# deezer/musicFPaugment

Measured on AMD Instinct MI355X. Metric: 8s/8kHz clips/sec (STFT+UNet+peak-pick), higher is better.
Workload: dtype bf16x3 (fp32 operands split into bf16 hi+lo, fp32 accumulate); 1 GPU; STFT(512/256,f64) -> UNet(1,1) eval forward (bf16x3 MFMA, formula weights) -> Audfprint peak-pick; 8 s / 8 kHz clips, 257x251 spectrograms; parallelism=clip-sharded x1, no data-path collective

## Files before the change

### musicfpaugment_amd/csrc/unet_wd16.hip

```cpp
#include "mfpa_common.h"
#include "mfpa_conv_tile.h"
#include "mfpa_unet_args.h"

namespace {

using namespace mfpa_tile;
using mfpa_unet::ConvArgs;

constexpr int wd16_bn(int wmw) { return 32 * (8 / wmw); }
constexpr bool wd16_persist(bool rows, int wmw, bool side, bool plain) { return wmw == 4 || (!rows && !side) || plain; }
template <int PH, int PW, bool IN16>
struct Wd16Lds {
  static constexpr int THREADS = 512;
  static constexpr int SPP = IN16 ? KC / 8 : KC / 4;
  static constexpr int HPW = PW + 2, HPH = PH + 2, HP = HPW * HPH;
  static constexpr int A_F4 = (HP * SPP + THREADS - 1) / THREADS;
  static constexpr int HPS = A_F4 * (THREADS / SPP);
  static constexpr int PLANE = ((HPS * 16 + 255) / 256) * 256;
  static constexpr int HLS = 4 * PLANE + 256;
  static constexpr int STAGE = 2 * HLS;
  static constexpr int TBL = 2 * A_F4 * THREADS;
  static constexpr int TBL_BYTES = 2 * ((HP * (KC / 4) + THREADS - 1) / THREADS) * THREADS * (int)sizeof(unsigned);
  static constexpr int RED = 2 * 256;
  static constexpr int epi_floats(int wmw) { return 2 * wd16_bn(wmw) + 64; }
  static constexpr int fixed_bytes(int wmw) { return 2 * STAGE + TBL_BYTES + epi_floats(wmw) * (int)sizeof(float); }
  __host__ __device__ static constexpr int plane_off(int hl, int kg) { return hl * HLS + kg * PLANE + (kg >> 1) * 128; }
  static_assert(TBL * (int)sizeof(unsigned) <= TBL_BYTES, "the kernel's table fits the launcher's");
};
static_assert(Wd16Lds<8, 32, false>::fixed_bytes(2) == 125184 && Wd16Lds<16, 16, false>::fixed_bytes(2) == 125184 &&
              Wd16Lds<8, 32, true>::fixed_bytes(2) == 125184 && Wd16Lds<16, 16, true>::fixed_bytes(2) == 125184, "LDS of the 128-channel tiles");
static_assert(Wd16Lds<8, 32, false>::fixed_bytes(4) == 124672 && Wd16Lds<8, 32, true>::fixed_bytes(4) == 124672, "LDS of the 64-channel tiles");


template <int PH, int PW, bool ROWS, int WMW = 2, bool SIDE = false, bool PLAIN = false, bool IN16 = false, bool AFF16 = false>
__global__ __launch_bounds__(512, 1) void conv_wd16_kernel(ConvArgs a) {
  static_assert(!IN16 || PLAIN, "a bf16 source feeds the plain-bf16 products");
  using G = Wd16Lds<PH, PW, IN16>;
  constexpr int SPP = G::SPP, HPW = G::HPW, HP = G::HP, A_F4 = G::A_F4, HLS = G::HLS, STAGE = G::STAGE, TBL = G::TBL;
  constexpr int ESZ = IN16 ? 2 : 4;
  constexpr int THREADS = G::THREADS, BN = wd16_bn(WMW), WPXW = 256 / WMW, TAPS = 9;
  static_assert((WMW == 2 || WMW == 4) && (!ROWS || WMW == 2), "wave grid");
  constexpr int BM = PH * PW;
  static_assert(BM == 256 && (PW == 32 || PW == 16), "two waves of 128 pixels: eight 16-pixel tiles each");
  constexpr int PT = WPXW / 16;
  static_assert(A_F4 <= TAPS - 3, "one halo staging slot per tap, taps 2 .. 7");

  extern __shared__ __attribute__((aligned(16))) char smem[];
  const int tid = threadIdx.x, lane = tid & 63, wave = tid >> 6;
  const int wm = wave % WMW, wn = __builtin_amdgcn_readfirstlane(wave / WMW);
  const int p = lane & 15, g = lane >> 4;

  constexpr bool PERSIST = wd16_persist(ROWS, WMW, SIDE, PLAIN);
  const int n0 = blockIdx.y * BN;
  const int Cin = a.C0 + a.C1;
  const int nchunks = Cin / KC;
  const int ntiles = a.tiles_x * a.tiles_y * a.B;

  const int aq = tid % SPP;
  unsigned* const aoffs0 = reinterpret_cast<unsigned*>(smem + 2 * STAGE);
#pragma unroll
  for (int it = 0; it < A_F4; ++it) {
    const int pix = tid / SPP + it * (THREADS / SPP);
    const int py = pix / HPW - 1, px = pix % HPW - 1;
    aoffs0[it * THREADS + tid] = (unsigned)((py * a.W + px) * a.C0 + (KC / SPP) * aq) * (unsigned)ESZ;
    aoffs0[(A_F4 + it) * THREADS + tid] = (unsigned)(((py - a.oy1) * a.W1 + (px - a.ox1)) * a.C1 + (KC / SPP) * aq) * (unsigned)ESZ;
  }
  const unsigned clip0 = (unsigned)a.H * (unsigned)a.W * (unsigned)a.C0 * (unsigned)ESZ, clip1 = (unsigned)a.H1 * (unsigned)a.W1 * (unsigned)a.C1 * (unsigned)ESZ;
  struct Tile { int b, y0, x0p; unsigned ain; unsigned t0, t1; };
  auto make_tile = [&](int t) __attribute__((always_inline)) {
    Tile T;
    int bx = __builtin_amdgcn_readfirstlane(t);
    const int tx = bx % a.tiles_x; bx /= a.tiles_x;
    const int ty = bx % a.tiles_y; bx /= a.tiles_y;
    T.b = bx; T.y0 = ty * PH; T.x0p = tx * PW; T.ain = 0;
    T.t0 = (unsigned)((T.y0 * a.W + T.x0p) * a.C0) * (unsigned)ESZ;
    T.t1 = (unsigned)((T.y0 * a.W1 + T.x0p) * a.C1) * (unsigned)ESZ;
#pragma unroll
    for (int it = 0; it < A_F4; ++it) {
      const int pix = tid / SPP + it * (THREADS / SPP);
      const int gy = T.y0 + pix / HPW - 1, gx = T.x0p + pix % HPW - 1;
      const bool in = pix < HP && gy >= 0 && gy < a.H && gx >= 0 && gx < a.W;
      const int y1 = gy - a.oy1, x1 = gx - a.ox1;
      const bool in1 = in && y1 >= 0 && y1 < a.H1 && x1 >= 0 && x1 < a.W1;
      T.ain |= (in ? 1u : 0u) << it | (in1 ? 1u : 0u) << (8 + it);
    }
    return T;
  };
  auto clip_rsrc = [&](const float* base, int b, unsigned clip_bytes) __attribute__((always_inline)) {
    const char* pb = reinterpret_cast<const char*>(base) + (size_t)b * clip_bytes;
    return __builtin_amdgcn_make_buffer_rsrc(const_cast<char*>(pb), 0, base != nullptr ? (int)clip_bytes : 0, 0x00020000);
  };
  int tile = blockIdx.x;
  Tile S = make_tile(tile);
  int eb = S.b, ey0 = S.y0, ex0p = S.x0p;
  float* aff = reinterpret_cast<float*>(smem + 2 * STAGE + TBL * sizeof(unsigned));
  if (a.in_scale0 != nullptr) {
    for (int i = tid; i < a.C0; i += THREADS) {
      aff[i] = a.in_scale0[i];
      aff[a.C0 + i] = a.in_shift0[i];
    }
    __syncthreads();
  }
  float* const epi = aff + (a.in_scale0 ? 2 * a.C0 : 0) + (a.w1x1 ? G::RED : 0);
  for (int i = tid; i < BN; i += THREADS) {
    epi[i] = a.scale ? a.scale[n0 + i] : 1.f;
    epi[BN + i] = a.shift ? a.shift[n0 + i] : 0.f;
  }
  if (a.w1x1 != nullptr && tid < 64) epi[2 * BN + tid] = a.w1x1[tid];
  constexpr int AHALF = (A_F4 + 1) / 2, AREGS = ROWS ? AHALF : A_F4;
  f32x4 areg[AREGS];
  auto load_a_range = [&](int chunk, auto FIRST, auto COUNT) __attribute__((always_inline)) {
    constexpr int first = decltype(FIRST)::value, count = decltype(COUNT)::value;
    const int c0 = chunk * KC;
    const bool from0 = c0 < a.C0;
    const auto rs = clip_rsrc(from0 ? a.x0 : a.x1, S.b, from0 ? clip0 : clip1);
    const unsigned toff = from0 ? S.t0 + (unsigned)c0 * (unsigned)ESZ : S.t1 + (unsigned)(c0 - a.C0) * (unsigned)ESZ;
    const unsigned* ao = aoffs0 + (from0 ? 0 : A_F4 * THREADS) + tid;
#pragma unroll
    for (int it = first; it < first + count && it < A_F4; ++it)
      areg[it % AREGS] = __builtin_bit_cast(f32x4, __builtin_amdgcn_raw_buffer_load_b128(rs, (int)(ao[it * THREADS] + toff), 0, 0));
  };
  auto load_a = [&](int chunk) __attribute__((always_inline)) {
    load_a_range(chunk, std::integral_constant<int, 0>{}, std::integral_constant<int, AREGS>{});
  };
  auto preload_offsets = [&](int chunk) __attribute__((always_inline)) {
    const unsigned* ao = aoffs0 + (chunk * KC < a.C0 ? 0 : A_F4 * THREADS) + tid;
#pragma unroll
    for (int it = 0; it < A_F4; ++it) areg[it % AREGS][0] = __uint_as_float(ao[it * THREADS]);
  };
  auto load_a_pre = [&](int chunk) __attribute__((always_inline)) {
    const int c0 = chunk * KC;
    const bool from0 = c0 < a.C0;
    const auto rs = clip_rsrc(from0 ? a.x0 : a.x1, S.b, from0 ? clip0 : clip1);
    const unsigned toff = from0 ? S.t0 + (unsigned)c0 * (unsigned)ESZ : S.t1 + (unsigned)(c0 - a.C0) * (unsigned)ESZ;
#pragma unroll
    for (int it = 0; it < A_F4; ++it)
      areg[it % AREGS] = __builtin_bit_cast(f32x4, __builtin_amdgcn_raw_buffer_load_b128(rs, (int)(__float_as_uint(areg[it % AREGS][0]) + toff), 0, 0));
  };
  auto split_slot = [&](auto IT, int chunk, char* stage) __attribute__((always_inline)) {
    constexpr int it = decltype(IT)::value;
    const int pix = tid / SPP + it * (THREADS / SPP);
    const int c0 = chunk * KC;
    const bool inside = (S.ain >> ((c0 < a.C0 ? 0 : 8) + it)) & 1u;
    f32x4 v = areg[it % AREGS];
    if (!inside) v = f32x4{0.f, 0.f, 0.f, 0.f};
    if constexpr (IN16) {
      if (AFF16 && a.in_scale0 != nullptr && c0 < a.C0 && inside) {
        float f[8];
#pragma unroll
        for (int k = 0; k < 4; ++k) {
          const unsigned u = __float_as_uint(v[k]);
          f[2 * k] = __uint_as_float(u << 16);
          f[2 * k + 1] = __uint_as_float(u & 0xffff0000u);
        }
        const float* scp = aff + c0 + 8 * aq;
        const float* shp = aff + a.C0 + c0 + 8 * aq;
        const f32x4 sc0 = *reinterpret_cast<const f32x4*>(scp), sc1 = *reinterpret_cast<const f32x4*>(scp + 4);
        const f32x4 sh0 = *reinterpret_cast<const f32x4*>(shp), sh1 = *reinterpret_cast<const f32x4*>(shp + 4);
#pragma unroll
        for (int k = 0; k < 8; ++k) {
          const float y = f[k] * (k < 4 ? sc0[k & 3] : sc1[k & 3]) + (k < 4 ? sh0[k & 3] : sh1[k & 3]);
          f[k] = y > 0.f ? y : 0.f;
        }
        if (a.drop_thresh) {
          const int gy = S.y0 + pix / HPW - 1, gx = S.x0p + pix % HPW - 1;
          const unsigned long long e0 = (((unsigned long long)S.b * a.H + gy) * a.W + gx) * a.C0 + c0 + 8 * aq;
#pragma unroll
          for (int k = 0; k < 8; ++k) f[k] = mfpa_keep(a.drop_seed, a.drop_thresh, e0 + k) ? f[k] * a.drop_scale : 0.f;
        }
#pragma unroll
        for (int k = 0; k < 4; ++k) {
          bf16x2 h2;
          h2[0] = (__bf16)f[2 * k];
          h2[1] = (__bf16)f[2 * k + 1];
          v[k] = __builtin_bit_cast(float, h2);
        }
      }
      *reinterpret_cast<f32x4*>(stage + G::plane_off(0, aq) + pix * 16) = v;
      if constexpr (SIDE && AFF16) {
        const int py = pix / HPW, px = pix % HPW;
        if (a.x0_bf16 != nullptr && c0 < a.C0 && inside && py >= 1 && py <= PH && px >= 1 && px <= PW && blockIdx.y == 0) {
          const size_t e = (size_t)S.b * a.H * a.W * a.C0 + ((aoffs0[it * THREADS + tid] + S.t0) >> 1) + c0;
          *reinterpret_cast<f32x4*>(a.x0_bf16 + e) = v;
        }
      }
      return;
    }
    if (a.in_scale0 != nullptr && c0 < a.C0 && inside) {
      const f32x4 sc = *reinterpret_cast<const f32x4*>(aff + c0 + 4 * aq);
      const f32x4 sh = *reinterpret_cast<const f32x4*>(aff + a.C0 + c0 + 4 * aq);
      v = v * sc + sh;
#pragma unroll
      for (int k = 0; k < 4; ++k) v[k] = v[k] > 0.f ? v[k] : 0.f;
      if (a.drop_thresh) {
        const int gy = S.y0 + pix / HPW - 1, gx = S.x0p + pix % HPW - 1;
        const unsigned long long e0 = (((unsigned long long)S.b * a.H + gy) * a.W + gx) * a.C0 + c0 + 4 * aq;
#pragma unroll
        for (int k = 0; k < 4; ++k) v[k] = mfpa_keep(a.drop_seed, a.drop_thresh, e0 + k) ? v[k] * a.drop_scale : 0.f;
      }
    }
    bf16x4 hi, lo;
#pragma unroll
    for (int k = 0; k < 4; ++k) {
      hi[k] = (__bf16)v[k];
      lo[k] = (__bf16)(v[k] - (float)hi[k]);
    }
    char* at = stage + G::plane_off(0, aq >> 1) + pix * 16 + 8 * (aq & 1);
    *reinterpret_cast<bf16x4*>(at) = hi;
    if constexpr (!PLAIN) *reinterpret_cast<bf16x4*>(at + HLS) = lo;
    if constexpr (SIDE) {
      const int py = pix / HPW, px = pix % HPW;
      const bool interior = inside && py >= 1 && py <= PH && px >= 1 && px <= PW && blockIdx.y == 0;
      if (a.x0_bf16 != nullptr && c0 < a.C0 && interior) {
        const size_t e = (size_t)S.b * a.H * a.W * a.C0 + ((aoffs0[it * THREADS + tid] + S.t0) >> 2) + c0;
        *reinterpret_cast<bf16x4*>(a.x0_bf16 + e) = hi;
      }
      if (a.x1_bf16 != nullptr && c0 >= a.C0 && interior) {
        const size_t e = (size_t)S.b * a.H1 * a.W1 * a.C1 + ((aoffs0[(A_F4 + it) * THREADS + tid] + S.t1) >> 2) + (c0 - a.C0);
        *reinterpret_cast<bf16x4*>(a.x1_bf16 + e) = hi;
      }
    }
  };

  bf16x8 wq[3][2][2];
  auto w_frag = [&](int tap, int chunk) __attribute__((always_inline)) {
    return reinterpret_cast<const char*>(a.w) +
           ((((size_t)tap * nchunks + chunk) * (size_t)(a.Cout / 16) + (size_t)(n0 / 16 + 2 * wn)) << 11) + lane * 16;
  };
  auto load_w = [&](int chunk, int tap, auto SLOT) __attribute__((always_inline)) {
    constexpr int slot = decltype(SLOT)::value;
    const char* wb = w_frag(tap, chunk);
    wq[slot][0][0] = *reinterpret_cast<const bf16x8*>(wb);
    if constexpr (!PLAIN) wq[slot][0][1] = *reinterpret_cast<const bf16x8*>(wb + 1024);
    wq[slot][1][0] = *reinterpret_cast<const bf16x8*>(wb + 2048);
    if constexpr (!PLAIN) wq[slot][1][1] = *reinterpret_cast<const bf16x8*>(wb + 3072);
  };

  struct XFrags { bf16x8 h[4], l[4]; };
  XFrags fx0, fx1;
  const int xbase = (((wm * WPXW + p) / PW) * HPW + ((wm * WPXW + p) % PW)) * 16 + G::plane_off(0, g);
  auto tile_disp = [](int pt) { return (PW == 32) ? ((pt >> 1) * HPW + (pt & 1) * 16) * 16 : pt * HPW * 16; };
  auto read_x = [&](XFrags& f, const char* stage, int tap_off, int half) __attribute__((always_inline)) {
#pragma unroll
    for (int i = 0; i < 4; ++i) {
      const char* r = stage + xbase + tile_disp(4 * half + i) + tap_off;
      if constexpr (!PLAIN) f.l[i] = *reinterpret_cast<const bf16x8*>(r + HLS);
      f.h[i] = *reinterpret_cast<const bf16x8*>(r);
    }
  };
  floatx4 acc[2][PT];
#pragma unroll
  for (int ct = 0; ct < 2; ++ct)
#pragma unroll
    for (int pt = 0; pt < PT; ++pt) acc[ct][pt] = floatx4{0.f, 0.f, 0.f, 0.f};
  auto mfma_half = [&](const XFrags& f, const bf16x8 (&w)[2][2], int half) __attribute__((always_inline)) {
    if constexpr (!PLAIN) {
#pragma unroll
    for (int ct = 0; ct < 2; ++ct)
#pragma unroll
      for (int i = 0; i < 4; ++i) acc[ct][4 * half + i] = __builtin_amdgcn_mfma_f32_16x16x32_bf16(w[ct][1], f.h[i], acc[ct][4 * half + i], 0, 0, 0);
#pragma unroll
    for (int ct = 0; ct < 2; ++ct)
#pragma unroll
      for (int i = 0; i < 4; ++i) acc[ct][4 * half + i] = __builtin_amdgcn_mfma_f32_16x16x32_bf16(w[ct][0], f.l[i], acc[ct][4 * half + i], 0, 0, 0);
    }
#pragma unroll
    for (int ct = 0; ct < 2; ++ct)
#pragma unroll
      for (int i = 0; i < 4; ++i) acc[ct][4 * half + i] = __builtin_amdgcn_mfma_f32_16x16x32_bf16(w[ct][0], f.h[i], acc[ct][4 * half + i], 0, 0, 0);
  };
  using S0 = std::integral_constant<int, 0>;
  using S1 = std::integral_constant<int, 1>;
  constexpr int N_R = PLAIN ? 4 : 8, N_M = PLAIN ? 8 : 24;
  constexpr int N_W = PLAIN ? 2 : 4;
  auto tap_body = [&](auto TAP, int chunk) __attribute__((always_inline)) {
    constexpr int tap = decltype(TAP)::value;
    constexpr int ntap = (tap + 1) % TAPS;
    constexpr int tap_off = ((tap / 3) * HPW + (tap % 3)) * 16, ntap_off = ((ntap / 3) * HPW + (ntap % 3)) * 16;
    const int chunk_n = chunk + 1 < nchunks ? chunk + 1 : (PERSIST ? 0 : chunk);
    const char* cur = smem + (chunk & 1) * STAGE;
    const char* nxt = (tap == TAPS - 1) ? smem + ((chunk + 1) & 1) * STAGE : cur;
    read_x(fx1, cur, tap_off, 1);
    mfma_half(fx0, wq[tap % 3], 0);
    load_w((tap + 2 >= TAPS) ? chunk_n : chunk, (tap + 2) % TAPS, std::integral_constant<int, (tap + 2) % 3>{});
    pin_reads<N_M - 1, N_R>();
    constexpr int used_a = pin_read_slots(N_M - 1, N_R);
    __builtin_amdgcn_sched_group_barrier(0x008, 1, 0);
    __builtin_amdgcn_sched_group_barrier(0x020, N_W, 0);
    if constexpr (N_M - used_a - 1 > 0) __builtin_amdgcn_sched_group_barrier(0x008, N_M - used_a - 1, 0);
    __builtin_amdgcn_sched_barrier(0);
    if (tap == TAPS - 1) {
      __syncthreads();
      __builtin_amdgcn_sched_barrier(0);
    }
    if (tap == 0) load_a_pre(chunk_n);
    if (tap == TAPS - 1) preload_offsets(PERSIST ? (chunk + 2 < nchunks ? chunk + 2 : chunk + 1 < nchunks ? 0 : 1 < nchunks ? 1 : 0)
                                                 : (chunk + 2 < nchunks ? chunk + 2 : chunk + 1 < nchunks ? chunk + 1 : chunk));
    read_x(fx0, nxt, ntap_off, 0);
    mfma_half(fx1, wq[tap % 3], 1);
    if constexpr (tap >= 2 && tap - 2 < A_F4) {
      split_slot(std::integral_constant<int, tap - 2>{}, chunk_n, smem + ((chunk + 1) & 1) * STAGE);
#pragma unroll
      for (int i = 0; i < N_R; ++i) {
        __builtin_amdgcn_sched_group_barrier(0x008, 1, 0);
        __builtin_amdgcn_sched_group_barrier(0x100, 1, 0);
        __builtin_amdgcn_sched_group_barrier(0x002, 2, 0);
      }
#pragma unroll
      for (int i = 0; i < 2; ++i) {
        __builtin_amdgcn_sched_group_barrier(0x008, 2, 0);
        __builtin_amdgcn_sched_group_barrier(0x002, 4, 0);
        __builtin_amdgcn_sched_group_barrier(0x200, 1, 0);
      }
      if constexpr (N_M - N_R - 4 > 0) __builtin_amdgcn_sched_group_barrier(0x008, N_M - N_R - 4, 0);
    } else {
      pin_reads<N_M, N_R>();
      if constexpr (N_M - pin_read_slots(N_M, N_R) > 0) __builtin_amdgcn_sched_group_barrier(0x008, N_M - pin_read_slots(N_M, N_R), 0);
    }
    __builtin_amdgcn_sched_barrier(0);
  };

  auto tap_body4 = [&](auto TAP, auto PAR, int chunk) __attribute__((always_inline)) {
    constexpr int tap = decltype(TAP)::value, par = (decltype(PAR)::value + tap) & 1;
    constexpr int ntap = (tap + 1) % TAPS;
    constexpr int ntap_off = ((ntap / 3) * HPW + (ntap % 3)) * 16;
    const int chunk_n = chunk + 1 < nchunks ? chunk + 1 : 0;
    const char* cur = smem + (chunk & 1) * STAGE;
    const char* nxt = (tap == TAPS - 1) ? smem + ((chunk + 1) & 1) * STAGE : cur;
    if (tap == TAPS - 1) {
      __syncthreads();
      __builtin_amdgcn_sched_barrier(0);
    }
    if (tap == 0) load_a_pre(chunk_n);
    if (tap == TAPS - 1) preload_offsets(chunk + 2 < nchunks ? chunk + 2 : chunk + 1 < nchunks ? 0 : 1 < nchunks ? 1 : 0);
    read_x(par ? fx0 : fx1, nxt, ntap_off, 0);
    mfma_half(par ? fx1 : fx0, wq[tap % 3], 0);
    load_w((tap + 2 >= TAPS) ? chunk_n : chunk, (tap + 2) % TAPS, std::integral_constant<int, (tap + 2) % 3>{});
    if constexpr (tap >= 2 && tap - 2 < A_F4) {
      split_slot(std::integral_constant<int, tap - 2>{}, chunk_n, smem + ((chunk + 1) & 1) * STAGE);
#pragma unroll
      for (int i = 0; i < N_R; ++i) {
        __builtin_amdgcn_sched_group_barrier(0x008, 1, 0);
        __builtin_amdgcn_sched_group_barrier(0x100, 1, 0);
        __builtin_amdgcn_sched_group_barrier(0x002, 2, 0);
      }
#pragma unroll
      for (int i = 0; i < N_W; ++i) {
        if constexpr (!PLAIN) __builtin_amdgcn_sched_group_barrier(0x008, 1, 0);
        __builtin_amdgcn_sched_group_barrier(0x020, 1, 0);
        __builtin_amdgcn_sched_group_barrier(0x002, 2, 0);
      }
#pragma unroll
      for (int i = 0; i < 2; ++i) {
        __builtin_amdgcn_sched_group_barrier(0x008, 2, 0);
        __builtin_amdgcn_sched_group_barrier(0x002, 4, 0);
        __builtin_amdgcn_sched_group_barrier(0x200, 1, 0);
      }
      if constexpr (N_M - N_R - 8 > 0) __builtin_amdgcn_sched_group_barrier(0x008, N_M - N_R - 8, 0);
    } else {
#pragma unroll
      for (int i = 0; i < N_R; ++i) {
        __builtin_amdgcn_sched_group_barrier(0x008, 1, 0);
        __builtin_amdgcn_sched_group_barrier(0x100, 1, 0);
      }
#pragma unroll
      for (int i = 0; i < N_W; ++i) {
        __builtin_amdgcn_sched_group_barrier(0x008, 1, 0);
        __builtin_amdgcn_sched_group_barrier(0x020, 1, 0);
      }
      if constexpr (N_M - N_R - N_W > 0) __builtin_amdgcn_sched_group_barrier(0x008, N_M - N_R - N_W, 0);
    }
    __builtin_amdgcn_sched_barrier(0);
  };

  constexpr int R = BM / 2 / PW, HV = PW / 16;
  bf16x8 wr[2][3][2][2];
  constexpr int NU = (R + 2) * HV, NB = (PW == 32) ? 4 : 5;
  static_assert(NU % NB == 0, "static ring indices");
  auto load_wr1 = [&](int chunk, auto DX, auto PAR, auto DY) __attribute__((always_inline)) {
    constexpr int dx = decltype(DX)::value, par = decltype(PAR)::value, dy = decltype(DY)::value;
    const char* wb = w_frag(dy * 3 + dx, chunk);
    wr[par][dy][0][0] = *reinterpret_cast<const bf16x8*>(wb);
    if constexpr (!PLAIN) wr[par][dy][0][1] = *reinterpret_cast<const bf16x8*>(wb + 1024);
    wr[par][dy][1][0] = *reinterpret_cast<const bf16x8*>(wb + 2048);
    if constexpr (!PLAIN) wr[par][dy][1][1] = *reinterpret_cast<const bf16x8*>(wb + 3072);
  };
  struct XUnit { bf16x8 h, l; };
  XUnit xu[NB];
  auto read_unit = [&](XUnit& f, const char* stage, int u, int dx) __attribute__((always_inline)) {
    const char* r = stage + xbase + ((u / HV) * HPW + (u % HV) * 16 + dx) * 16;
    if constexpr (!PLAIN) f.l = *reinterpret_cast<const bf16x8*>(r + HLS);
    f.h = *reinterpret_cast<const bf16x8*>(r);
  };
  auto mfma_unit = [&](auto U, const XUnit& f, auto PAR) __attribute__((always_inline)) {
    constexpr int h = decltype(U)::value / HV, hv = decltype(U)::value % HV, par = decltype(PAR)::value;
#pragma unroll
    for (int term = PLAIN ? 2 : 0; term < 3; ++term)
#pragma unroll
      for (int dy = 0; dy < 3; ++dy) {
        if (h - dy < 0 || h - dy >= R) continue;
#pragma unroll
        for (int ct = 0; ct < 2; ++ct) {
          floatx4& c = acc[ct][(h - dy) * HV + hv];
          c = __builtin_amdgcn_mfma_f32_16x16x32_bf16(wr[par][dy][ct][term == 0 ? 1 : 0], term == 1 ? f.l : f.h, c, 0, 0, 0);
        }
      }
  };
  auto unit_mfmas = [](int u) { const int h = u / HV; int n = 0; for (int dy = 0; dy < 3; ++dy) n += (h - dy >= 0 && h - dy < R) ? 1 : 0; return n * (PLAIN ? 2 : 6); };
  constexpr int BARU = NU - NB + 1;
  constexpr int SA = NU / 2, SB = BARU - AHALF;
  static_assert(SA + AHALF < NU && SB >= 0, "staging schedule");
  auto unit_step = [&](auto U, auto DX, auto PAR, int chunk) __attribute__((always_inline)) {
    constexpr int u = decltype(U)::value, dx = decltype(DX)::value, par = decltype(PAR)::value;
    constexpr int n_m = unit_mfmas(u);
    const int chunk_n = chunk + 1 < nchunks ? chunk + 1 : (PERSIST ? 0 : chunk);
    const char* cur = smem + (chunk & 1) * STAGE;
    char* nxs = smem + ((chunk + 1) & 1) * STAGE;
    if constexpr (u == BARU && dx == 2) {
      __syncthreads();
      __builtin_amdgcn_sched_barrier(0);
    }
    constexpr int pu = u + NB - 1;
    if constexpr (pu < NU) read_unit(xu[pu % NB], cur, pu, dx);
    else read_unit(xu[pu % NB], dx == 2 ? nxs : cur, pu - NU, (dx + 1) % 3);
    mfma_unit(U, xu[u % NB], PAR);
    constexpr int split_it = dx == 1 ? u - SA : dx == 2 ? AHALF + u - SB : -1;
    constexpr bool do_split = (dx == 1 && u >= SA && u < SA + AHALF) || (dx == 2 && u >= SB && u < SB + AHALF && split_it < A_F4);
    if constexpr (u == 0 && dx == 0) load_a_range(chunk_n, std::integral_constant<int, 0>{}, std::integral_constant<int, AHALF>{});
    if constexpr (u == SA + AHALF && dx == 1) load_a_range(chunk_n, std::integral_constant<int, AHALF>{}, std::integral_constant<int, AHALF>{});
    if constexpr (u >= 1 && u <= 3) {
      if constexpr (dx < 2) load_wr1(chunk, std::integral_constant<int, (dx + 1) % 3>{}, std::integral_constant<int, par ^ 1>{}, std::integral_constant<int, u - 1>{});
      else load_wr1(chunk_n, std::integral_constant<int, 0>{}, std::integral_constant<int, par ^ 1>{}, std::integral_constant<int, u - 1>{});
    }
    if constexpr (do_split) split_slot(std::integral_constant<int, split_it>{}, chunk_n, nxs);
    __builtin_amdgcn_sched_group_barrier(0x008, 1, 0);
    __builtin_amdgcn_sched_group_barrier(0x100, PLAIN ? 1 : 2, 0);
    if constexpr (do_split && PLAIN) {
#pragma unroll
      for (int i = 1; i < n_m; ++i) {
        __builtin_amdgcn_sched_group_barrier(0x002, (24 + n_m - 2) / (n_m - 1), 0);
        __builtin_amdgcn_sched_group_barrier(0x008, 1, 0);
      }
      __builtin_amdgcn_sched_group_barrier(0x200, 1, 0);
    } else if constexpr (PLAIN && u >= 1 && u <= 3) {
      __builtin_amdgcn_sched_group_barrier(0x020, 2, 0);
      if constexpr (n_m - 1 > 0) __builtin_amdgcn_sched_group_barrier(0x008, n_m - 1, 0);
    } else if constexpr (do_split) {
      __builtin_amdgcn_sched_group_barrier(0x002, 6, 0);
#pragma unroll
      for (int i = 0; i < 4; ++i) {
        __builtin_amdgcn_sched_group_barrier(0x008, 1, 0);
        __builtin_amdgcn_sched_group_barrier(0x002, 6, 0);
      }
      __builtin_amdgcn_sched_group_barrier(0x200, 2, 0);
      if constexpr (n_m - 5 > 0) __builtin_amdgcn_sched_group_barrier(0x008, n_m - 5, 0);
    } else if constexpr (u >= 1 && u <= 3) {
#pragma unroll
      for (int i = 0; i < 4; ++i) {
        __builtin_amdgcn_sched_group_barrier(0x008, 1, 0);
        __builtin_amdgcn_sched_group_barrier(0x020, 1, 0);
      }
      if constexpr (n_m - 5 > 0) __builtin_amdgcn_sched_group_barrier(0x008, n_m - 5, 0);
    } else {
      if constexpr (n_m - 1 > 0) __builtin_amdgcn_sched_group_barrier(0x008, n_m - 1, 0);
    }
    __builtin_amdgcn_sched_barrier(0);
  };
  auto period = [&](auto DX, auto PAR, int chunk) __attribute__((always_inline)) {
    each_index<NU>(unit_step, DX, PAR, chunk);
  };

  if constexpr (ROWS) {
    f32x4 keep[AREGS];
    load_a_range(0, std::integral_constant<int, AHALF>{}, std::integral_constant<int, AHALF>{});
#pragma unroll
    for (int i = 0; i < AREGS; ++i) keep[i] = areg[i];
    load_a_range(0, std::integral_constant<int, 0>{}, std::integral_constant<int, AHALF>{});
    each_index<3>([&](auto DY) __attribute__((always_inline)) { load_wr1(0, S0{}, S0{}, DY); });
    each_index<AHALF>(split_slot, 0, smem);
#pragma unroll
    for (int i = 0; i < AREGS; ++i) areg[i] = keep[i];
    each_index<A_F4 - AHALF, AHALF>(split_slot, 0, smem);
    static_assert(A_F4 <= 2 * AHALF, "two halves of staging slots");
  } else {
    load_a(0);
    load_w(0, 0, S0{});
    load_w(0, 1, S1{});
    each_index<A_F4>(split_slot, 0, smem);
    preload_offsets(1 < nchunks ? 1 : 0);
  }
  auto epilogue = [&]() __attribute__((always_inline)) {
  #pragma unroll
    for (int ct = 0; ct < 2; ++ct) {
      const int chl = wn * 32 + ct * 16 + 4 * g;
      const f32x4 sc = *reinterpret_cast<const f32x4*>(epi + chl);
      const f32x4 sh = *reinterpret_cast<const f32x4*>(epi + BN + chl);
  #pragma unroll
      for (int pt = 0; pt < PT; ++pt)
  #pragma unroll
        for (int j = 0; j < 4; ++j) {
          float v = acc[ct][pt][j] * sc[j] + sh[j];
          if (a.relu) v = v > 0.f ? v : 0.f;
          acc[ct][pt][j] = v;
        }
    }
    if (SIDE && a.stats_part != nullptr) {
      float vm[PT];
  #pragma unroll
      for (int pt = 0; pt < PT; ++pt) {
        const int m = wm * WPXW + pt * 16 + p;
        vm[pt] = (ey0 + m / PW < a.yH && ex0p + m % PW < a.yW) ? 1.f : 0.f;
      }
      float* row = a.stats_part + ((size_t)tile * WMW + wm) * 2 * a.Cout + n0 + wn * 32 + 4 * g;
  #pragma unroll
      for (int ct = 0; ct < 2; ++ct) {
        f32x4 sv = {0.f, 0.f, 0.f, 0.f}, qv = {0.f, 0.f, 0.f, 0.f};
        if (!AFF16 && a.bz != nullptr) {
          const int ch = n0 + wn * 32 + ct * 16 + 4 * g;
          const f32x4 bsc = *reinterpret_cast<const f32x4*>(a.bz_scale + ch), bsh = *reinterpret_cast<const f32x4*>(a.bz_shift + ch);
          const f32x4 bmu = *reinterpret_cast<const f32x4*>(a.bz_mean + ch), bis = *reinterpret_cast<const f32x4*>(a.bz_invstd + ch);
          f32x4 zzs[PT];
          auto zoff = [&](int pt) __attribute__((always_inline)) {
            const int m = wm * WPXW + pt * 16 + p;
            const int gy = min(ey0 + m / PW, a.yH - 1), gx = min(ex0p + m % PW, a.yW - 1);
            return (((size_t)eb * a.yH + gy) * a.yW + gx) * (size_t)a.Cout + ch;
          };
          if (a.bz16) {
            f32x2 raw[PT];
  #pragma unroll
            for (int pt = 0; pt < PT; ++pt) raw[pt] = *reinterpret_cast<const f32x2*>(reinterpret_cast<const __bf16*>(a.bz) + zoff(pt));
  #pragma unroll
            for (int pt = 0; pt < PT; ++pt) {
              const unsigned u0 = __float_as_uint(raw[pt][0]), u1 = __float_as_uint(raw[pt][1]);
              zzs[pt] = f32x4{__uint_as_float(u0 << 16), __uint_as_float(u0 & 0xffff0000u), __uint_as_float(u1 << 16), __uint_as_float(u1 & 0xffff0000u)};
            }
          } else {
  #pragma unroll
            for (int pt = 0; pt < PT; ++pt) zzs[pt] = *reinterpret_cast<const f32x4*>(a.bz + zoff(pt));
          }
  #pragma unroll
          for (int pt = 0; pt < PT; ++pt) {
            const f32x4 zz = zzs[pt];
  #pragma unroll
            for (int j = 0; j < 4; ++j) {
              const float gg = (zz[j] * bsc[j] + bsh[j] > 0.f) ? acc[ct][pt][j] * vm[pt] : 0.f;
              sv[j] += gg;
              qv[j] += gg * ((zz[j] - bmu[j]) * bis[j]);
            }
          }
        } else {
  #pragma unroll
        for (int pt = 0; pt < PT; ++pt)
  #pragma unroll
          for (int j = 0; j < 4; ++j) {
            const float v = acc[ct][pt][j] * vm[pt];
            sv[j] += v;
            qv[j] += v * v;
          }
        }
  #pragma unroll
        for (int j = 0; j < 4; ++j) {
          sv[j] = dpp_row_add<0x118>(dpp_row_add<0x114>(dpp_row_add<0x112>(dpp_row_add<0x111>(sv[j]))));
          qv[j] = dpp_row_add<0x118>(dpp_row_add<0x114>(dpp_row_add<0x112>(dpp_row_add<0x111>(qv[j]))));
        }
        if (p == 15) {
          *reinterpret_cast<f32x4*>(row + ct * 16) = sv;
          *reinterpret_cast<f32x4*>(row + a.Cout + ct * 16) = qv;
        }
      }
    }
    if (a.y != nullptr || (SIDE && IN16 && a.y_bf16 != nullptr)) {
      char* yb = reinterpret_cast<char*>(a.y + (size_t)eb * a.yH * a.yW * a.Cout);
  #pragma unroll
      for (int pt = 0; pt < PT; ++pt) {
        const int m = wm * WPXW + pt * 16 + p;
        const int gy = ey0 + m / PW, gx = ex0p + m % PW;
        if (gy < a.yH && gx < a.yW) {
          char* yp = yb + (((unsigned)gy * (unsigned)a.yW + (unsigned)gx) * (unsigned)a.Cout + (unsigned)(n0 + wn * 32 + 4 * g)) * 4u;
          if (a.y != nullptr) {
  #pragma unroll
          for (int ct = 0; ct < 2; ++ct) {
            f32x4 o;
  #pragma unroll
            for (int j = 0; j < 4; ++j) o[j] = acc[ct][pt][j];
            *reinterpret_cast<f32x4*>(yp + ct * 64) = o;
          }
          }
          if (SIDE && a.y_bf16 != nullptr) {
            __bf16* hp = a.y_bf16 + (((size_t)eb * a.yH + gy) * a.yW + gx) * (size_t)a.Cout + n0 + wn * 32 + 4 * g;
  #pragma unroll
            for (int ct = 0; ct < 2; ++ct) {
              bf16x4 h;
  #pragma unroll
              for (int j = 0; j < 4; ++j) h[j] = (__bf16)acc[ct][pt][j];
              *reinterpret_cast<bf16x4*>(hp + ct * 16) = h;
            }
          }
        }
      }
    }
    if (a.y_pool != nullptr) {
      const int Ho = a.H / 2, Wo = a.W / 2;
      constexpr int ROWSTEP = (PW == 32) ? 2 : 1;
  #pragma unroll
      for (int ct = 0; ct < 2; ++ct)
  #pragma unroll
        for (int pt = 0; pt < PT; ++pt) {
          const int row = pt / ROWSTEP;
          if (row & 1) continue;
          f32x4 v;
  #pragma unroll
          for (int j = 0; j < 4; ++j) {
            const float t = fmaxf(acc[ct][pt][j], acc[ct][pt + ROWSTEP][j]);
            const float o = __int_as_float(__builtin_amdgcn_update_dpp(0, __float_as_int(t), 0xB1, 0xf, 0xf, true));
            v[j] = fmaxf(t, o);
          }
          const int m = wm * WPXW + pt * 16 + p;
          const int py = (ey0 + m / PW) / 2, px = (ex0p + m % PW) / 2;
          if (!(p & 1) && py < Ho && px < Wo)
            *reinterpret_cast<f32x4*>(a.y_pool + (((size_t)eb * Ho + py) * Wo + px) * a.Cout + n0 + wn * 32 + ct * 16 + 4 * g) = v;
        }
    }
  
    if constexpr (WMW == 4) {
      if (a.w1x1 != nullptr) {
        float* red = reinterpret_cast<float*>(smem + 2 * STAGE + TBL * sizeof(unsigned)) + (a.in_scale0 ? 2 * a.C0 : 0);
        const f32x4 w0 = *reinterpret_cast<const f32x4*>(epi + 2 * BN + wn * 32 + 4 * g);
        const f32x4 w1 = *reinterpret_cast<const f32x4*>(epi + 2 * BN + wn * 32 + 16 + 4 * g);
  #pragma unroll
        for (int pt = 0; pt < PT; ++pt) {
          float v = 0.f;
  #pragma unroll
          for (int j = 0; j < 4; ++j) v += acc[0][pt][j] * w0[j] + acc[1][pt][j] * w1[j];
          v += __shfl_xor(v, 16);
          v += __shfl_xor(v, 32);
          if (g == 0) red[wn * 256 + wm * WPXW + pt * 16 + p] = v;
        }
        __syncthreads();
        if (tid < 256) {
          const int gy = ey0 + tid / PW, gx = ex0p + tid % PW;
          if (gy < a.H && gx < a.W) a.y1x1[((size_t)eb * a.H + gy) * a.W + gx] = red[tid] + red[256 + tid] + a.b1x1;
        }
        __syncthreads();
      }
    }
  };

  __syncthreads();
  if constexpr (ROWS) {
#pragma unroll
    for (int u = 0; u < NB - 1; ++u) read_unit(xu[u], smem, u, 0);
  } else {
    read_x(fx0, smem, 0, 0);
  }
  for (;;) {
    const int tile_n = tile + (int)gridDim.x;
    const bool has_next = PERSIST && tile_n < ntiles;
    const Tile N = PERSIST ? make_tile(has_next ? tile_n : tile) : S;
    if constexpr (ROWS) {
      using D0 = std::integral_constant<int, 0>;
      using D1 = std::integral_constant<int, 1>;
      using D2 = std::integral_constant<int, 2>;
      for (int chunk = 0; chunk < nchunks; chunk += 2) {
        period(D0{}, S0{}, chunk);
        period(D1{}, S1{}, chunk);
        period(D2{}, S0{}, chunk);
        if (PERSIST && chunk + 2 >= nchunks) S = N;
        period(D0{}, S1{}, chunk + 1);
        period(D1{}, S0{}, chunk + 1);
        period(D2{}, S1{}, chunk + 1);
      }
    } else if constexpr (WMW == 4) {
      for (int chunk = 0; chunk < nchunks; chunk += 2) {
        each_index<TAPS>(tap_body4, S0{}, chunk);
        if (chunk + 2 >= nchunks) S = N;
        each_index<TAPS>(tap_body4, S1{}, chunk + 1);
      }
    } else {
      for (int chunk = 0; chunk < nchunks; ++chunk) {
        if (PERSIST && chunk + 1 >= nchunks) S = N;
        each_index<TAPS>(tap_body, chunk);
      }
    }
    epilogue();
    if (!has_next) break;
    tile = tile_n; eb = S.b; ey0 = S.y0; ex0p = S.x0p;
#pragma unroll
    for (int ct = 0; ct < 2; ++ct)
#pragma unroll
      for (int pt = 0; pt < PT; ++pt) acc[ct][pt] = floatx4{0.f, 0.f, 0.f, 0.f};
  }
}

}

namespace mfpa_unet {

const int CONV_WD16_ROWS = 512;
void conv_wd16_tile(int W, int Cout, mfpa_conv_route* t) {
  t->wmw = Cout % 128 ? 4 : 2; t->bn = 32 * (8 / t->wmw);
  t->pw = (t->wmw == 2 && W <= 16) ? 16 : 32; t->ph = 256 / t->pw;
}

template <int PH, int PW, bool ROWS, int WMW, bool SIDE, bool PLAIN, bool IN16, bool AFF16>
int launch_wd16(ConvArgs& a, hipStream_t s) {
  using G = Wd16Lds<PH, PW, IN16>;
  const size_t lds = (size_t)G::fixed_bytes(WMW) +
                     (a.in_scale0 ? (size_t)2 * a.C0 * sizeof(float) : 0) +
                     (a.w1x1 ? G::RED * sizeof(float) : 0);
  dim3 grid((unsigned)((long long)a.tiles_x * a.tiles_y * a.B), (unsigned)(a.Cout / wd16_bn(WMW)));
  if constexpr (wd16_persist(ROWS, WMW, SIDE, PLAIN)) {
    const int cus = mfpa_current_device_cus();
    const unsigned per = (unsigned)((cus > 0 ? cus : 256) / (int)grid.y);
    if (per >= 1 && grid.x > per && ((a.C0 + a.C1) / KC) % 2 == 0) grid.x = per;
  }
  hipLaunchKernelGGL((conv_wd16_kernel<PH, PW, ROWS, WMW, SIDE, PLAIN, IN16, AFF16>), grid, dim3(G::THREADS), lds, s, a);
  MFPA_CHECK_LAUNCH();
  return MFPA_OK;
}
#define MFPA_WD16_INSTANTIATE(...) template int launch_wd16<__VA_ARGS__>(ConvArgs&, hipStream_t);
MFPA_WD16_FORMS(MFPA_WD16_INSTANTIATE)

}
```

Measured before the change: 5279 clips/s.

## De-interleave halo columns in wd16 conv to share LDS fragment reads across taps

For the non-row, two-wave-column, 32-wide, non-side configuration, the halo row is stored with even and odd columns de-interleaved (reusing the role-split kernels' layout). Each wave's 16-pixel tile then covers every other pixel, so fragments read for one horizontal tap can be partly reused by the next tap, and only half of the A reads need to be reissued. The accumulator-to-pixel mapping, output store indexing and the 2x2 max-pool epilogue are rewritten to match, and a new tap schedule with tuned sched_group_barriers is added. This aims to cut LDS read traffic per tap. The cost is more complex index mapping and a dependence on the role_split halo_col layout.

```diff
diff --git a/musicfpaugment_amd/csrc/unet_wd16.hip b/musicfpaugment_amd/csrc/unet_wd16.hip
--- a/musicfpaugment_amd/csrc/unet_wd16.hip
+++ b/musicfpaugment_amd/csrc/unet_wd16.hip
@@ -51,6 +51,9 @@
   const int p = lane & 15, g = lane >> 4;
 
   constexpr bool PERSIST = wd16_persist(ROWS, WMW, SIDE, PLAIN);
+  constexpr bool SHARE = !ROWS && WMW == 2 && PW == 32 && !SIDE;
+  static_assert(!SHARE || (HPW == role_split::HPW && PH == role_split::PH), "the de-interleaved halo row of the role-split kernels");
+  auto hcol = [](int pos) { return SHARE ? role_split::halo_col(pos) : pos; };
   const int n0 = blockIdx.y * BN;
   const int Cin = a.C0 + a.C1;
   const int nchunks = Cin / KC;
@@ -61,7 +64,7 @@
 #pragma unroll
   for (int it = 0; it < A_F4; ++it) {
     const int pix = tid / SPP + it * (THREADS / SPP);
-    const int py = pix / HPW - 1, px = pix % HPW - 1;
+    const int py = pix / HPW - 1, px = hcol(pix % HPW) - 1;
     aoffs0[it * THREADS + tid] = (unsigned)((py * a.W + px) * a.C0 + (KC / SPP) * aq) * (unsigned)ESZ;
     aoffs0[(A_F4 + it) * THREADS + tid] = (unsigned)(((py - a.oy1) * a.W1 + (px - a.ox1)) * a.C1 + (KC / SPP) * aq) * (unsigned)ESZ;
   }
@@ -78,7 +81,7 @@
 #pragma unroll
     for (int it = 0; it < A_F4; ++it) {
       const int pix = tid / SPP + it * (THREADS / SPP);
-      const int gy = T.y0 + pix / HPW - 1, gx = T.x0p + pix % HPW - 1;
+      const int gy = T.y0 + pix / HPW - 1, gx = T.x0p + hcol(pix % HPW) - 1;
       const bool in = pix < HP && gy >= 0 && gy < a.H && gx >= 0 && gx < a.W;
       const int y1 = gy - a.oy1, x1 = gx - a.ox1;
       const bool in1 = in && y1 >= 0 && y1 < a.H1 && x1 >= 0 && x1 < a.W1;
@@ -193,7 +196,7 @@
 #pragma unroll
       for (int k = 0; k < 4; ++k) v[k] = v[k] > 0.f ? v[k] : 0.f;
       if (a.drop_thresh) {
-        const int gy = S.y0 + pix / HPW - 1, gx = S.x0p + pix % HPW - 1;
+        const int gy = S.y0 + pix / HPW - 1, gx = S.x0p + hcol(pix % HPW) - 1;
         const unsigned long long e0 = (((unsigned long long)S.b * a.H + gy) * a.W + gx) * a.C0 + c0 + 4 * aq;
 #pragma unroll
         for (int k = 0; k < 4; ++k) v[k] = mfpa_keep(a.drop_seed, a.drop_thresh, e0 + k) ? v[k] * a.drop_scale : 0.f;
@@ -238,7 +241,8 @@
 
   struct XFrags { bf16x8 h[4], l[4]; };
   XFrags fx0, fx1;
-  const int xbase = (((wm * WPXW + p) / PW) * HPW + ((wm * WPXW + p) % PW)) * 16 + G::plane_off(0, g);
+  const int xbase = SHARE ? ((wm * (WPXW / PW)) * HPW + p) * 16 + G::plane_off(0, g)
+                          : (((wm * WPXW + p) / PW) * HPW + ((wm * WPXW + p) % PW)) * 16 + G::plane_off(0, g);
   auto tile_disp = [](int pt) { return (PW == 32) ? ((pt >> 1) * HPW + (pt & 1) * 16) * 16 : pt * HPW * 16; };
   auto read_x = [&](XFrags& f, const char* stage, int tap_off, int half) __attribute__((always_inline)) {
 #pragma unroll
@@ -248,26 +252,37 @@
       f.h[i] = *reinterpret_cast<const bf16x8*>(r);
     }
   };
+  constexpr int R_ALL = 0, R_FIRST = 1, R_SECOND = 2;
+  auto read_set = [&](XFrags& f, const char* stage, auto TA, auto SET, auto PART) __attribute__((always_inline)) {
+    constexpr int ta = decltype(TA)::value, s = decltype(SET)::value, part = decltype(PART)::value;
+#pragma unroll
+    for (int j = (part == R_SECOND ? 2 : 0); j < (part == R_FIRST ? 2 : 4); ++j) {
+      const char* r = stage + xbase + ((ta + j) * HPW + (s & 1) * role_split::HALF + (s >> 1)) * 16;
+      if constexpr (!PLAIN) f.l[j] = *reinterpret_cast<const bf16x8*>(r + HLS);
+      f.h[j] = *reinterpret_cast<const bf16x8*>(r);
+    }
+  };
   floatx4 acc[2][PT];
 #pragma unroll
   for (int ct = 0; ct < 2; ++ct)
 #pragma unroll
     for (int pt = 0; pt < PT; ++pt) acc[ct][pt] = floatx4{0.f, 0.f, 0.f, 0.f};
+  auto half_pt = [](int half, int i) { return SHARE ? 2 * i + half : 4 * half + i; };
   auto mfma_half = [&](const XFrags& f, const bf16x8 (&w)[2][2], int half) __attribute__((always_inline)) {
     if constexpr (!PLAIN) {
 #pragma unroll
     for (int ct = 0; ct < 2; ++ct)
 #pragma unroll
-      for (int i = 0; i < 4; ++i) acc[ct][4 * half + i] = __builtin_amdgcn_mfma_f32_16x16x32_bf16(w[ct][1], f.h[i], acc[ct][4 * half + i], 0, 0, 0);
+      for (int i = 0; i < 4; ++i) acc[ct][half_pt(half, i)] = __builtin_amdgcn_mfma_f32_16x16x32_bf16(w[ct][1], f.h[i], acc[ct][half_pt(half, i)], 0, 0, 0);
 #pragma unroll
     for (int ct = 0; ct < 2; ++ct)
 #pragma unroll
-      for (int i = 0; i < 4; ++i) acc[ct][4 * half + i] = __builtin_amdgcn_mfma_f32_16x16x32_bf16(w[ct][0], f.l[i], acc[ct][4 * half + i], 0, 0, 0);
+      for (int i = 0; i < 4; ++i) acc[ct][half_pt(half, i)] = __builtin_amdgcn_mfma_f32_16x16x32_bf16(w[ct][0], f.l[i], acc[ct][half_pt(half, i)], 0, 0, 0);
     }
 #pragma unroll
     for (int ct = 0; ct < 2; ++ct)
 #pragma unroll
-      for (int i = 0; i < 4; ++i) acc[ct][4 * half + i] = __builtin_amdgcn_mfma_f32_16x16x32_bf16(w[ct][0], f.h[i], acc[ct][4 * half + i], 0, 0, 0);
+      for (int i = 0; i < 4; ++i) acc[ct][half_pt(half, i)] = __builtin_amdgcn_mfma_f32_16x16x32_bf16(w[ct][0], f.h[i], acc[ct][half_pt(half, i)], 0, 0, 0);
   };
   using S0 = std::integral_constant<int, 0>;
   using S1 = std::integral_constant<int, 1>;
@@ -320,6 +335,64 @@
     __builtin_amdgcn_sched_barrier(0);
   };
 
+  auto tap_share = [&](auto TAP, int chunk) __attribute__((always_inline)) {
+    constexpr int tap = decltype(TAP)::value, ta = tap / 3, tb = tap % 3;
+    using TA = std::integral_constant<int, ta>;
+    using I0 = std::integral_constant<int, 0>;
+    using RAll = std::integral_constant<int, R_ALL>;
+    using PartA = std::integral_constant<int, tb == 0 ? R_ALL : R_SECOND>;
+    constexpr int n_ra = tb == 0 ? N_R : N_R / 2, n_rb = tb == 2 ? N_R : N_R / 2;
+    const int chunk_n = chunk + 1 < nchunks ? chunk + 1 : (PERSIST ? 0 : chunk);
+    const char* cur = smem + (chunk & 1) * STAGE;
+    XFrags& fa = (tb & 1) ? fx1 : fx0;
+    XFrags& fb = (tb & 1) ? fx0 : fx1;
+    read_set(fb, cur, TA{}, std::integral_constant<int, tb + 1>{}, PartA{});
+    mfma_half(fa, wq[tap % 3], 0);
+    load_w((tap + 2 >= TAPS) ? chunk_n : chunk, (tap + 2) % TAPS, std::integral_constant<int, (tap + 2) % 3>{});
+    pin_reads<N_M - 1, n_ra>();
+    constexpr int used_a = pin_read_slots(N_M - 1, n_ra);
+    __builtin_amdgcn_sched_group_barrier(0x008, 1, 0);
+    __builtin_amdgcn_sched_group_barrier(0x020, N_W, 0);
+    if constexpr (N_M - used_a - 1 > 0) __builtin_amdgcn_sched_group_barrier(0x008, N_M - used_a - 1, 0);
+    __builtin_amdgcn_sched_barrier(0);
+    if constexpr (tap == TAPS - 1) {
+      __syncthreads();
+      __builtin_amdgcn_sched_barrier(0);
+    }
+    if constexpr (tap == 0) load_a_pre(chunk_n);
+    if constexpr (tap == TAPS - 1) preload_offsets(PERSIST ? (chunk + 2 < nchunks ? chunk + 2 : chunk + 1 < nchunks ? 0 : 1 < nchunks ? 1 : 0)
+                                                           : (chunk + 2 < nchunks ? chunk + 2 : chunk + 1 < nchunks ? chunk + 1 : chunk));
+    if constexpr (tap == TAPS - 1) read_set(fa, smem + ((chunk + 1) & 1) * STAGE, I0{}, I0{}, RAll{});
+    else if constexpr (tb == 2) read_set(fa, cur, std::integral_constant<int, ta + 1>{}, I0{}, RAll{});
+    else read_set(fa, cur, TA{}, std::integral_constant<int, tb + 2>{}, std::integral_constant<int, R_FIRST>{});
+    mfma_half(fb, wq[tap % 3], 1);
+    if constexpr (tap >= 2 && tap - 2 < A_F4) {
+      split_slot(std::integral_constant<int, tap - 2>{}, chunk_n, smem + ((chunk + 1) & 1) * STAGE);
+#pragma unroll
+      for (int i = 0; i < n_rb; ++i) {
+        __builtin_amdgcn_sched_group_barrier(0x008, 1, 0);
+        __builtin_amdgcn_sched_group_barrier(0x100, 1, 0);
+        __builtin_amdgcn_sched_group_barrier(0x002, 2, 0);
+      }
+#pragma unroll
+      for (int i = n_rb; i < N_R; ++i) {
+        __builtin_amdgcn_sched_group_barrier(0x008, 1, 0);
+        __builtin_amdgcn_sched_group_barrier(0x002, 2, 0);
+      }
+#pragma unroll
+      for (int i = 0; i < 2; ++i) {
+        __builtin_amdgcn_sched_group_barrier(0x008, 2, 0);
+        __builtin_amdgcn_sched_group_barrier(0x002, 4, 0);
+        __builtin_amdgcn_sched_group_barrier(0x200, 1, 0);
+      }
+      if constexpr (N_M - N_R - 4 > 0) __builtin_amdgcn_sched_group_barrier(0x008, N_M - N_R - 4, 0);
+    } else {
+      pin_reads<N_M, n_rb>();
+      if constexpr (N_M - pin_read_slots(N_M, n_rb) > 0) __builtin_amdgcn_sched_group_barrier(0x008, N_M - pin_read_slots(N_M, n_rb), 0);
+    }
+    __builtin_amdgcn_sched_barrier(0);
+  };
+
   auto tap_body4 = [&](auto TAP, auto PAR, int chunk) __attribute__((always_inline)) {
     constexpr int tap = decltype(TAP)::value, par = (decltype(PAR)::value + tap) & 1;
     constexpr int ntap = (tap + 1) % TAPS;
@@ -573,7 +646,7 @@
       char* yb = reinterpret_cast<char*>(a.y + (size_t)eb * a.yH * a.yW * a.Cout);
   #pragma unroll
       for (int pt = 0; pt < PT; ++pt) {
-        const int m = wm * WPXW + pt * 16 + p;
+        const int m = SHARE ? (wm * (WPXW / PW) + (pt >> 1)) * PW + 2 * p + (pt & 1) : wm * WPXW + pt * 16 + p;
         const int gy = ey0 + m / PW, gx = ex0p + m % PW;
         if (gy < a.yH && gx < a.yW) {
           char* yp = yb + (((unsigned)gy * (unsigned)a.yW + (unsigned)gx) * (unsigned)a.Cout + (unsigned)(n0 + wn * 32 + 4 * g)) * 4u;
@@ -602,6 +675,20 @@
     if (a.y_pool != nullptr) {
       const int Ho = a.H / 2, Wo = a.W / 2;
       constexpr int ROWSTEP = (PW == 32) ? 2 : 1;
+      if constexpr (SHARE) {
+  #pragma unroll
+        for (int ct = 0; ct < 2; ++ct)
+  #pragma unroll
+          for (int r = 0; r < PT / 2; r += 2) {
+            f32x4 v;
+  #pragma unroll
+            for (int j = 0; j < 4; ++j)
+              v[j] = fmaxf(fmaxf(acc[ct][2 * r][j], acc[ct][2 * r + 2][j]), fmaxf(acc[ct][2 * r + 1][j], acc[ct][2 * r + 3][j]));
+            const int py = (ey0 + wm * (WPXW / PW) + r) / 2, px = ex0p / 2 + p;
+            if (py < Ho && px < Wo)
+              *reinterpret_cast<f32x4*>(a.y_pool + (((size_t)eb * Ho + py) * Wo + px) * a.Cout + n0 + wn * 32 + ct * 16 + 4 * g) = v;
+          }
+      } else {
   #pragma unroll
       for (int ct = 0; ct < 2; ++ct)
   #pragma unroll
@@ -620,6 +707,7 @@
           if (!(p & 1) && py < Ho && px < Wo)
             *reinterpret_cast<f32x4*>(a.y_pool + (((size_t)eb * Ho + py) * Wo + px) * a.Cout + n0 + wn * 32 + ct * 16 + 4 * g) = v;
         }
+      }
     }
   
     if constexpr (WMW == 4) {
@@ -650,6 +738,8 @@
   if constexpr (ROWS) {
 #pragma unroll
     for (int u = 0; u < NB - 1; ++u) read_unit(xu[u], smem, u, 0);
+  } else if constexpr (SHARE) {
+    read_set(fx0, smem, S0{}, S0{}, std::integral_constant<int, R_ALL>{});
   } else {
     read_x(fx0, smem, 0, 0);
   }
@@ -679,7 +769,8 @@
     } else {
       for (int chunk = 0; chunk < nchunks; ++chunk) {
         if (PERSIST && chunk + 1 >= nchunks) S = N;
-        each_index<TAPS>(tap_body, chunk);
+        if constexpr (SHARE) each_index<TAPS>(tap_share, chunk);
+        else each_index<TAPS>(tap_body, chunk);
       }
     }
     epilogue();
```

Result: no change. 5268 clips/s (-0.2%).
